# JiQi-da/Mixed-Graph-ADMM

Hardware: AMD Instinct MI355X
Metric: ADMM iters/sec x batch (sample-iterations/s) (higher is better)
Workload: dtype f32; 1 GPU; cfg2: PEMS04-shaped synthetic graph N=307 (path+chords, 340 edges), kNN k=4, T=24, t_in=12; batch_per_gpu=4096, global_batch=4096, ablation=None, graph=kNN-directed, max_cg_iter=100, parallelism=batch-sharded x1, no collective on the convergence path, final RCCL gather, all_finite=True

## Files before the change

mixed-graph-admm_amd/csrc/lds_args.h:

```cpp
#pragma once
#include <hip/hip_runtime.h>

#include "lds_consts.h"
#include "lds_param_table.h"
#include "lds_adapt.h"

struct LdsArgsCore {
    int T, N, TN, TS, t_in, G, B, Bp;
    int nthreads;
    int NR;
    int has_phi, has_zd, first;
    int J;
    int lhsx_kind;
    int band, skip, q1;
    int max_cg;
    int record;
    int stagger_wgs, stagger_ticks;
    int tail_pairs;
    float rho, rho_u, rho_d, mu_u, mu_d1, mu_d2;
    float cx1, cx2;
    double cg_tol2;
    const int* csr;
    int lds_img0, lds_img_ints;
    int off_rp_u, off_rp_d, off_en_u, off_en_d, off_lead_t, off_tail_t;
    int off_diag;
    const float* band_w;
    float *zu, *zd, *phi, *gam, *gu, *gd;
    const float* y;
    const float* mask;
    double* ps;
    int* cg_iters;
    float* alpha_hist;
    float* beta_hist;
    int* nonfinite;
    const int* stop;
};
struct LdsArgs : LdsArgsCore {
    float* xs[LDS_MAXJ + 1];
    int* pstop;
    int* pstop_count;
    float* x_final;
    double admm_tol;
    int it0;
    const LdsSampleParams* sp;
    unsigned long long npos;
    int off_node;
    int img_stride;
    const int* gset;
    int sp_rows{}, sp_row0{}, sp_stride{};
};

struct LdsLaunch {
    int64_t key;
    int block;
    size_t lds_bytes;
    int64_t* instance;
    int* unit;
};

int mg_lds_iteration(const LdsLaunch& L, const LdsArgs& a, int B, hipStream_t st);
int mg_lds_iteration_ps(const LdsLaunch& L, const LdsArgs& a, int B, hipStream_t st);
int mg_lds_iteration_pp(const LdsLaunch& L, const LdsArgs& a, int B, hipStream_t st);
int mg_lds_init(bool masked, int T, int t_in, int N, int TPG, int B, float tm, float den, const float* y, const float* mask, float* x,
                float* zu, float* zd, float* gam, float* gu, float* gd, int* nonfinite, const int* row_of_node, hipStream_t st);
int mg_lds_state_layout(bool to_thread_major, int T, int N, int TPG, int B, const float* src, float* dst, const int* row_of_node, hipStream_t st);
int mg_lds_dxps(int T, int N, int B, const float* x, const float* xo, double* scratch, double* out, const int* stop, hipStream_t st);
int mg_lds_ps_history(const double* ps, const int* pstop, int n_it, int max_it, int B, int Bp, int* n_per_sample, double* metrics,
                      double* out_ps, hipStream_t st);
int mg_lds_stop_test(const double* metrics_row, const int* nonfinite, int has_phi, int has_zd, double tol, int it, int* stop, hipStream_t st);
struct LdsAdaptArgs {
    const double* ps;
    const int* pstop;
    double* w;
    LdsSampleParams* table;
    double* hist;
    int B, Bp, row_first, row_last, ablation, has_phi, has_zd;
    ldsadapt::Params q;
};
int mg_lds_adapt(const LdsAdaptArgs& a, hipStream_t st);
```

mixed-graph-admm_amd/csrc/lds_engine.h:

```cpp
#pragma once
#include <thread>

#include "engine.h"
#include "lds_args.h"
#include "lds_graph_sets.h"
#include "lds_schedule.h"

namespace {

struct LdsEngine final : Engine<float> {
    int dev_cus = 0;
    int* d_lds_csr = nullptr;
    double* d_m2 = nullptr;
    int lds_async = 1;
    int* d_stop = nullptr;
    double* d_ps_ring = nullptr;
    int* d_pstop = nullptr;
    double* d_ps_full = nullptr;
    size_t ps_full_elems = 0;
    LdsSampleParams* d_sp = nullptr;
    LdsSampleParams* d_sch = nullptr;
    size_t sch_elems = 0;
    int sch_up_B = 0;
    LdsSampleParams* d_ad_tab = nullptr;
    double *d_ad_w = nullptr, *d_ad_hist = nullptr;
    size_t ad_tab_elems = 0, ad_w_elems = 0, ad_hist_elems = 0;
    int ad_last_B = 0;
    int* d_sg_img = nullptr;
    int* d_sg_set = nullptr;
    std::vector<int> lds_img_host;
    ldsplan::Switches lds_sw;
    static constexpr int ring_ids[] = {V_XA, V_XB, V_ZUB, V_ZDB, V_PHIB, V_Y, V_MASK, V_R, V_P, V_Q, V_AP, V_RHS, V_TMP, V_IO0, V_IO1};
    static constexpr int NRING = (int)(sizeof(ring_ids) / sizeof(ring_ids[0]));
    std::vector<float*> lds_ring_extra;
    hipStream_t st_side = nullptr;
    hipEvent_t ev_main[LDS_NBOUND] = {nullptr}, ev_side[LDS_NBOUND] = {nullptr};

    using Engine<float>::Engine;
    ~LdsEngine() override {
        (void)hipSetDevice(g->device);
        auto fr = [](void* q) { if (q) (void)hipFree(q); };
        fr(d_lds_csr); fr(d_m2); fr(d_stop); fr(d_ps_ring); fr(d_pstop); fr(d_ps_full);
        fr(d_sp); fr(d_sg_img); fr(d_sg_set); fr(d_sch); fr(d_ad_tab); fr(d_ad_w); fr(d_ad_hist);
        for (float* b : lds_ring_extra) if (b) (void)hipFree(b);
        if (st_side) (void)hipStreamDestroy(st_side);
        for (auto& e : ev_main) if (e) (void)hipEventDestroy(e);
        for (auto& e : ev_side) if (e) (void)hipEventDestroy(e);
    }

    int init() override {
        MG_TRY(init_workspace());
        if (const char* e = getenv("MGADMM_LDS_ASYNC")) lds_async = atoi(e);
        MG_TRY(plan_lds());
        return refused(solvegate::admm_convergence_gate(facts(p), "solver_create"));
    }

    int set_params(const mgadmm_params& np) override {
        const mgadmm_params old = p;
        const int rc = Engine<float>::set_params(np);
        if (p.rho != old.rho || p.rho_u != old.rho_u || p.rho_d != old.rho_d || p.mu_u != old.mu_u || p.mu_d1 != old.mu_d1 ||
            p.mu_d2 != old.mu_d2 || p.ablation != old.ablation)
            sch_up_B = 0;
        MG_TRY(rc);
        return wt.sp_B > 0 ? upload_sample_params(wt.sp_B) : (int)MGADMM_OK;
    }

    int set_sample_params(const mgadmm_sample_params* sp, int B) override {
        MG_TRY(Engine<float>::set_sample_params(sp, B));
        sch_up_B = 0;
        if (wt.sp_B == 0) return MGADMM_OK;
        MG_HIP(hipSetDevice(g->device));
        return upload_sample_params(wt.sp_B);
    }
    int upload_sample_params(int n) {
        std::vector<LdsSampleParams> rec;
        ldsparam::fill_records(wt.source(false, p), p.ablation, n, rec);
        if (!d_sp) MG_HIP(hipMalloc(&d_sp, sizeof(LdsSampleParams) * (size_t)Bmax));
        MG_HIP(hipMemcpy(d_sp, rec.data(), sizeof(LdsSampleParams) * rec.size(), hipMemcpyHostToDevice));
        return MGADMM_OK;
    }

    int set_param_schedule(const mgadmm_param_schedule* sch, int n_rows, int B, int first_row) override {
        MG_HIP(hipSetDevice(g->device));
        if ((sch == nullptr || n_rows == 0) && d_sch) {
            MG_HIP(hipDeviceSynchronize());
            (void)hipFree(d_sch);
            d_sch = nullptr;
            sch_elems = 0;
        }
        MG_TRY(Engine<float>::set_param_schedule(sch, n_rows, B, first_row));
        sch_up_B = 0;
        return MGADMM_OK;
    }
    int upload_param_schedule(int B) {
        if (sch_up_B == B && d_sch) return MGADMM_OK;
        std::vector<LdsSampleParams> rec;
        ldsparam::fill_records(wt.source(true, p), p.ablation, B, rec);
        MG_TRY(grow(d_sch, sch_elems, rec.size()));
        MG_HIP(hipMemcpy(d_sch, rec.data(), sizeof(LdsSampleParams) * rec.size(), hipMemcpyHostToDevice));
        sch_up_B = B;
        return MGADMM_OK;
    }

    int get_adaptive_history(int B, double* rho_hist, int max_periods, int* n_periods) override {
        MG_TRY(Engine<float>::get_adaptive_history(B, rho_hist, max_periods, n_periods));
        if (ad_last_periods == 0 || rho_hist == nullptr || max_periods <= 0) return MGADMM_OK;
        MG_REQUIRE(B == ad_last_B, "get_adaptive_history: the last adaptive_rho solve had B = %d, not %d", ad_last_B, B);
        MG_HIP(hipSetDevice(g->device));
        MG_HIP(hipMemcpy(rho_hist, d_ad_hist, sizeof(double) * 3 * (size_t)B * std::min(max_periods, ad_last_periods), hipMemcpyDeviceToHost));
        return MGADMM_OK;
    }

    int set_sample_graphs(int n_sets, mgadmm_graph* const* graphs, const int32_t* set_of_sample, int B) override {
        MG_HIP(hipSetDevice(g->device));
        if (n_sets == 0 && d_sg_img) {
            MG_HIP(hipDeviceSynchronize());
            (void)hipFree(d_sg_img);
            d_sg_img = nullptr;
        }
        MG_TRY(Engine<float>::set_sample_graphs(n_sets, graphs, set_of_sample, B));
        if (n_sets == 0) return MGADMM_OK;
        std::vector<ldsplan::Input> sets;
        for (int s = 0; s < n_sets; ++s)
            sets.push_back(ldsplan::Input{T, N, false, graphs[s]->transpose_by_gather != 0, graphs[s]->hWu, graphs[s]->hWd, graphs[s]->hWdT});
        std::vector<int> table;
        std::string differs;
        int bad = -1;
        if (!ldssets::build_table(lds, lds_img_host, sets, lds_sw, table, &bad, differs, std::min(8, (int)std::thread::hardware_concurrency()))) {
            mg_set_error("set_sample_graphs: sample_graphs set %d does not share the solver's topology -- %s (a weight that underflowed to 0 and "
                         "was dropped, another k or other neighbour lists?)", bad, differs.c_str());
            return MGADMM_ERR_UNSUPPORTED;
        }
        std::vector<int> set_of((size_t)Bp_max, 0);
        std::copy(set_of_sample, set_of_sample + B, set_of.begin());
        int* fresh = nullptr;
        MG_HIP(hipMalloc(&fresh, sizeof(int) * table.size()));
        if (hipMemcpy(fresh, table.data(), sizeof(int) * table.size(), hipMemcpyHostToDevice) != hipSuccess) {
            (void)hipFree(fresh);
            mg_set_error("set_sample_graphs: upload of the images failed");
            return MGADMM_ERR_HIP;
        }
        if (!d_sg_set) MG_HIP(hipMalloc(&d_sg_set, sizeof(int) * (size_t)Bp_max));
        MG_HIP(hipDeviceSynchronize());
        MG_HIP(hipMemcpy(d_sg_set, set_of.data(), sizeof(int) * set_of.size(), hipMemcpyHostToDevice));
        if (d_sg_img) (void)hipFree(d_sg_img);
        d_sg_img = fresh;
        sg_B = B;
        return MGADMM_OK;
    }

    int plan_lds() {
        if (hipDeviceGetAttribute(&dev_cus, hipDeviceAttributeMultiprocessorCount, g->device) != hipSuccess) { (void)hipGetLastError(); dev_cus = 0; }
        std::vector<int> img;
        const ldsplan::Input in{T, N, g->mode == MGADMM_TEMPORAL_BAND, g->transpose_by_gather != 0, g->hWu, g->hWd, g->hWdT};
        lds_sw = ldsplan::Switches::from_env();
        const ldsplan::Status planned = ldsplan::make(in, lds_sw, lds, img);
        if (planned == ldsplan::ROWS_DO_NOT_FIT) {
            mg_set_error("lds: row plan does not fit its launch word (%d waves)", lds.block / 64);
            return MGADMM_ERR_INVALID;
        }
        if (planned == ldsplan::NO_PLAN) return MGADMM_OK;
        MG_HIP(hipMalloc(&d_lds_csr, sizeof(int) * img.size()));
        MG_HIP(hipMemcpy(d_lds_csr, img.data(), sizeof(int) * img.size(), hipMemcpyHostToDevice));
        lds_img_host = img;
        MG_HIP(hipMalloc(&d_m2, sizeof(double) * T * N * (1 + (size_t)(Bmax + 63) / 64)));
        MG_HIP(hipMalloc(&d_stop, sizeof(int)));
        MG_HIP(hipMemset(d_stop, 0, sizeof(int)));
        MG_HIP(hipMalloc(&d_ps_ring, sizeof(double) * LDS_SETS * LDS_MAXJ * MGADMM_NMETRIC * Bp_max));
        MG_HIP(hipMalloc(&d_pstop, sizeof(int) * (2 * (size_t)Bp_max + 1)));
        {
            int lo = 0, hi = 0;
            MG_HIP(hipDeviceGetStreamPriorityRange(&lo, &hi));
            if (const char* e = getenv("MGADMM_LDS_SIDE_PRIO")) lo = atoi(e) > 0 ? hi : lo;
            MG_HIP(hipStreamCreateWithPriority(&st_side, hipStreamNonBlocking, lo));
            for (auto& e : ev_main) MG_HIP(hipEventCreateWithFlags(&e, hipEventDisableTiming));
            for (auto& e : ev_side) MG_HIP(hipEventCreateWithFlags(&e, hipEventDisableTiming));
        }
        return MGADMM_OK;
    }

    const int* lds_row_of_node() const { return lds.row_order ? d_lds_csr + lds.off_rown : nullptr; }

    int launch_lds(const LdsArgs& a, int B) {
        const bool timed = prof_open(0, 0.0);
        LdsLaunch L{lds.instance, lds.block, lds.lds_bytes, &lds_instance, &lds_unit};
        const int rc = mg_lds_iteration(L, a, B, st);
        if (timed) prof_close();
        return rc;
    }

    struct LdsRun {
        ldssched::Schedule s;
        LdsArgs a;
        int B, Bp;
        bool has_phi, has_zd, record, cold;
        float* xo;
        mgadmm_history* hist;
        int n_done = 0, rc = MGADMM_OK;
        std::vector<int> ad_bounds;
    };

    int lds_ring_reserve(int slots) {
        while (NRING + (int)lds_ring_extra.size() < slots) {
            float* b = nullptr;
            MG_HIP(hipMalloc(&b, vec_elems * sizeof(float)));
            lds_ring_extra.push_back(b);
            ws_bytes += (int64_t)(vec_elems * sizeof(float));
        }
        return MGADMM_OK;
    }
    float* lds_ring(int slot) const { return slot < NRING ? vec[ring_ids[slot]] : lds_ring_extra[slot - NRING]; }
    float* lds_xbuf(const LdsRun& r, int k) const {
        const int slot = r.s.slot_of_iterate(k);
        return slot == ldssched::X_OUT ? r.xo : lds_ring(slot);
    }

    void lds_fill_args(LdsRun& r, const void* y, const void* mask) const {
        LdsArgs& a = r.a;
        a = LdsArgs{};
        a.T = T; a.N = N; a.TN = T * N; a.TS = lds.TS; a.t_in = p.t_in; a.G = lds.G; a.B = r.B; a.Bp = r.Bp;
        a.nthreads = lds.nthreads; a.NR = lds.NR; a.tail_pairs = lds.tail_pairs;
        a.has_phi = r.has_phi; a.has_zd = r.has_zd;
        const LhsDef dx = lhs_def(MGADMM_LHS_X);
        a.lhsx_kind = dx.kind == 1 ? 1 : 0;
        a.cx1 = (float)dx.c1; a.cx2 = (float)dx.c2;
        a.band = g->mode == MGADMM_TEMPORAL_BAND; a.skip = g->skip;
        a.q1 = a.band ? 0 : g->q1;
        a.max_cg = p.max_cg_iter; a.record = r.record ? 1 : 0;
        a.rho = (float)p.rho; a.rho_u = (float)p.rho_u; a.rho_d = (float)p.rho_d;
        a.mu_u = (float)p.mu_u; a.mu_d1 = (float)p.mu_d1; a.mu_d2 = (float)p.mu_d2;
        a.cg_tol2 = p.cg_tol * p.cg_tol;
        a.csr = d_lds_csr; a.lds_img0 = lds.lds_img0; a.lds_img_ints = lds.lds_img_ints;
        a.off_rp_u = lds.off_rp_u; a.off_rp_d = lds.off_rp_d;
        a.off_en_u = lds.off_en_u; a.off_en_d = lds.off_en_d; a.off_lead_t = lds.off_lead_t; a.off_tail_t = lds.off_tail_t; a.off_diag = lds.off_diag;
        a.npos = lds.npos_word; a.off_node = lds.off_node;
        a.band_w = g->band_w;
        a.zu = vec[V_ZUA]; a.zd = vec[V_ZDA]; a.phi = vec[V_PHIA];
        a.gam = vec[V_GAM]; a.gu = vec[V_GU]; a.gd = vec[V_GD];
        const int ncu = dev_cus > 0 ? dev_cus : 256;
        int us = 48;
        if (const char* e = getenv("MGADMM_LDS_STAGGER_US")) us = atoi(e);
        a.stagger_wgs = ncu;
        a.stagger_ticks = (r.B >= 2 * ncu && us > 0) ? us * 100 : 0;
        a.y = (const float*)y; a.mask = (const float*)mask;
        a.alpha_hist = r.record ? d_alpha_hist : nullptr; a.beta_hist = r.record ? d_beta_hist : nullptr;
        a.nonfinite = d_nonfinite;
    }

    int lds_state_in(const LdsRun& r, const void* x0, const mgadmm_state* si) {
        const LdsArgs& a = r.a;
        float* const x = lds_xbuf(r, 0);
        if (!si) {
            float tm, den;
            time_moments(tm, den);
            return mg_lds_init(a.mask != nullptr, T, p.t_in, N, lds.TPG, r.B, tm, den, a.y, a.mask, x, a.zu, a.zd, a.gam, a.gu, a.gd,
                               d_nonfinite, lds_row_of_node(), st);
        }
        if (x0 != nullptr && x != x0) MG_HIP(hipMemcpyAsync(x, x0, (size_t)r.B * T * N * sizeof(float), hipMemcpyDeviceToDevice, st));
        auto in = [&](float* dst, const void* src) {
            return src == nullptr ? (int)MGADMM_OK : mg_lds_state_layout(true, T, N, lds.TPG, r.B, (const float*)src, dst, lds_row_of_node(), st);
        };
        MG_TRY(in(a.zu, si->zu));
        MG_TRY(in(a.gu, si->gamma_u));
        MG_TRY(in(a.zd, si->zd));
        MG_TRY(in(a.gd, si->gamma_d));
        MG_TRY(in(a.phi, si->phi));
        return in(a.gam, si->gamma);
    }
    int lds_state_out(const LdsRun& r, const mgadmm_state* so) {
        const LdsArgs& a = r.a;
        auto out = [&](void* dst, const float* src) {
            return dst == nullptr ? (int)MGADMM_OK : mg_lds_state_layout(false, T, N, lds.TPG, r.B, src, (float*)dst, lds_row_of_node(), st);
        };
        MG_TRY(out(so->zu, a.zu));
        MG_TRY(out(so->zd, a.zd));
        if (r.has_phi) {
            MG_TRY(out(so->phi, a.phi));
            MG_TRY(out(so->gamma, a.gam));
        }
        MG_TRY(out(so->gamma_u, a.gu));
        return out(so->gamma_d, a.gd);
    }

    int lds_batch_metrics(const LdsRun& r, int it, const double* ps, hipStream_t s) {
        const bool per_sample = r.hist && r.hist->metrics_per_sample;
        MG_TRY(mg_lds_dxps(T, N, r.B, lds_xbuf(r, it + 1), lds_xbuf(r, it), d_m2, d_dxps + (size_t)it * T, r.a.stop, s));
        hipLaunchKernelGGL(k_batch_metrics, dim3(MGADMM_NMETRIC), dim3(256), 0, s, ps, r.Bp, r.B, d_hist + (size_t)it * MGADMM_NMETRIC,
                           per_sample ? d_hist_ps + (size_t)it * MGADMM_NMETRIC * r.B : nullptr);
        MG_HIP(hipGetLastError());
        return MGADMM_OK;
    }

    int lagged_word(int c, const int* d_word, int* word) {
        const ldssched::LagStep l = ldssched::lag_step(c, LAG);
        MG_HIP(hipMemcpyAsync(h_flag + 1 + l.put, d_word, sizeof(int), hipMemcpyDeviceToHost, st));
        MG_HIP(hipEventRecord(ev_ring[l.put], st));
        *word = 0;
        if (l.get >= 0) {
            MG_HIP(hipEventSynchronize(ev_ring[l.get]));
            *word = h_flag[1 + l.get];
        }
        return MGADMM_OK;
    }

    int adapt_begin(LdsRun& r) {
        const int B = r.B, max_it = r.s.max_it;
        const ldsparam::Source src = wt.source(false, p);
        std::vector<LdsSampleParams> row, rec;
        ldsparam::fill_records(src, p.ablation, B, row);
        rec.reserve((size_t)max_it * B);
        for (int k = 0; k < max_it; ++k) rec.insert(rec.end(), row.begin(), row.end());
        std::vector<double> w((size_t)ldsparam::NW * B);
        for (int f = 0; f < ldsparam::NW; ++f)
            for (int b = 0; b < B; ++b) w[(size_t)f * B + b] = ldsparam::weight_of(src, f, 0, b);
        const size_t hist_rows = (size_t)max_it / ad.every + 2;
        MG_TRY(grow(d_ad_tab, ad_tab_elems, rec.size()));
        MG_TRY(grow(d_ad_w, ad_w_elems, w.size()));
        MG_TRY(grow(d_ad_hist, ad_hist_elems, hist_rows * 3 * B));
        MG_HIP(hipMemcpy(d_ad_tab, rec.data(), sizeof(LdsSampleParams) * rec.size(), hipMemcpyHostToDevice));
        MG_HIP(hipMemcpy(d_ad_w, w.data(), sizeof(double) * w.size(), hipMemcpyHostToDevice));
        MG_HIP(hipMemcpy(d_ad_hist, w.data(), sizeof(double) * 3 * B, hipMemcpyHostToDevice));
        MG_HIP(hipMemsetAsync(d_ad_hist + (size_t)3 * B, 0xFF, sizeof(double) * (hist_rows - 1) * 3 * B, st));
        ad_last_B = B;
        return MGADMM_OK;
    }
    int adapt_step(LdsRun& r, int it, const double* ps) {
        if (!ad_on || !ldsadapt::step_after(it, ad_start, ad.every, ad.until)) return MGADMM_OK;
        const ldsadapt::Rows rows = ldsadapt::rows_after(it, ad_start, ad.every, ad.until, r.s.max_it);
        r.ad_bounds.push_back(it + 1);
        LdsAdaptArgs k;
        k.ps = ps; k.pstop = r.a.pstop; k.w = d_ad_w; k.table = d_ad_tab;
        k.hist = d_ad_hist + r.ad_bounds.size() * 3 * (size_t)r.B;
        k.B = r.B; k.Bp = r.Bp; k.row_first = rows.first; k.row_last = rows.last;
        k.ablation = p.ablation; k.has_phi = r.has_phi; k.has_zd = r.has_zd;
        k.q = ad;
        return mg_lds_adapt(k, st);
    }

    int lds_run_chunks(LdsRun& r) {
        LdsArgs& a = r.a;
        const size_t row = (size_t)MGADMM_NMETRIC * r.Bp;
        int c = 0;
        for (; c < r.s.chunks(); ++c) {
            const ldssched::Chunk ch = r.s.chunk(c);
            a.first = ch.it0 == 0 && r.cold;
            a.J = ch.Jc;
            for (int k = 0; k <= ch.Jc; ++k) a.xs[k] = lds_xbuf(r, ch.it0 + k);
            a.cg_iters = d_cg_iters + (size_t)ch.it0 * 3 * r.Bp;
            a.it0 = ch.it0;
            if (r.s.per_sample) {
                a.ps = d_ps_full + (size_t)ch.it0 * row;
                MG_TRY(launch_lds(a, r.B));
                MG_TRY(adapt_step(r, ch.it0 + ch.Jc - 1, a.ps + (size_t)(ch.Jc - 1) * row));
                r.n_done = ch.it0 + ch.Jc;
                int stopped = 0;
                MG_TRY(lagged_word(c, a.pstop_count, &stopped));
                if (stopped == r.B) break;
                continue;
            }
            a.ps = d_ps_ring + (size_t)ch.set * r.s.J * row;
            if (ch.wait >= 0) MG_HIP(hipStreamWaitEvent(st, ev_side[ch.wait], 0));
            MG_TRY(launch_lds(a, r.B));
            MG_HIP(hipEventRecord(ev_main[ch.ev], st));
            MG_HIP(hipStreamWaitEvent(st_side, ev_main[ch.ev], 0));
            MG_TRY(adapt_step(r, ch.it0 + ch.Jc - 1, a.ps + (size_t)(ch.Jc - 1) * row));
            for (int k = 0; k < ch.Jc; ++k) MG_TRY(lds_batch_metrics(r, ch.it0 + k, a.ps + (size_t)k * row, st_side));
            MG_HIP(hipEventRecord(ev_side[ch.ev], st_side));
            r.n_done = ch.it0 + ch.Jc;
        }
        if (!r.s.per_sample && r.s.join(c) >= 0) MG_HIP(hipStreamWaitEvent(st, ev_side[r.s.join(c)], 0));
        return MGADMM_OK;
    }

    int lds_run_steps(LdsRun& r) {
        LdsArgs& a = r.a;
        const size_t K = p.max_cg_iter;
        for (int it = 0; it < r.s.max_it; ++it) {
            a.first = it == 0 && r.cold;
            a.J = 1;
            a.xs[0] = lds_xbuf(r, it); a.xs[1] = lds_xbuf(r, it + 1);
            a.cg_iters = d_cg_iters + (size_t)it * 3 * r.Bp;
            a.ps = d_ps;
            a.it0 = it;
            if (r.s.per_sample) a.ps = d_ps_full + (size_t)it * MGADMM_NMETRIC * r.Bp;
            if (r.record) {
                MG_TRY(fill(d_alpha_hist, 3 * K * r.Bp, (float)NAN));
                MG_TRY(fill(d_beta_hist, 3 * K * r.Bp, (float)NAN));
            }
            MG_TRY(launch_lds(a, r.B));
            MG_TRY(adapt_step(r, it, a.ps));
            if (!r.s.per_sample) MG_TRY(lds_batch_metrics(r, it, a.ps, st));
            if (r.record) {
                for (int w = 0; w < 3; ++w)
                    if (w < 2 || r.has_zd) MG_TRY(save_coeffs(r.Bp, r.hist, it, w, r.B, w));
            }
            r.n_done = it + 1;
            if (r.s.per_sample) {
                MG_HIP(hipMemcpyAsync(h_flag + 1, a.pstop_count, sizeof(int), hipMemcpyDeviceToHost, st));
                MG_HIP(hipStreamSynchronize(st));
                if (h_flag[1] == r.B) break;
            } else if (r.s.kind == ldssched::DEVSTOP) {
                int sw = 0;
                MG_TRY(mg_lds_stop_test(d_hist + (size_t)it * MGADMM_NMETRIC, d_nonfinite, r.has_phi, r.has_zd, p.admm_tol, it, d_stop, st));
                MG_TRY(lagged_word(it, d_stop, &sw));
                if (sw != 0) break;
            } else if (p.check_stop) {
                bool stop = false;
                MG_TRY(host_stop_test(it, r.has_phi, r.has_zd, &stop, &r.rc));
                if (stop) break;
            }
        }
        if (r.s.kind == ldssched::DEVSTOP) {
            MG_HIP(hipMemcpyAsync(h_flag + 1, d_stop, sizeof(int), hipMemcpyDeviceToHost, st));
            MG_HIP(hipStreamSynchronize(st));
            const int sw = h_flag[1];
            if (sw > 0) r.n_done = sw;
            else if (sw < 0) { r.n_done = -sw; r.rc = MGADMM_ERR_NONFINITE; }
        }
        return MGADMM_OK;
    }

    int lds_finish_per_sample(LdsRun& r, std::vector<int>& nps) {
        int* const d_nps = d_pstop + Bp_max + 1;
        MG_TRY(mg_lds_ps_history(d_ps_full, d_pstop, r.n_done, r.s.max_it, r.B, r.Bp, d_nps, d_hist,
                                 (r.hist && r.hist->metrics_per_sample) ? d_hist_ps : nullptr, st));
        nps.resize(r.B);
        MG_HIP(hipMemcpyAsync(nps.data(), d_nps, sizeof(int) * r.B, hipMemcpyDeviceToHost, st));
        MG_HIP(hipStreamSynchronize(st));
        r.n_done = *std::max_element(nps.begin(), nps.end());
        return MGADMM_OK;
    }

    int solve_lds(const void* y, const void* mask, int B, const void* x0, const mgadmm_state* state_in, void* x_out,
                  const mgadmm_state* state_out, mgadmm_history* hist) override {
        LdsRun r;
        r.B = B; r.Bp = (B + 63) / 64 * 64;
        r.has_phi = has_phi(); r.has_zd = has_zd();
        r.record = p.record_cg_coeffs && hist && hist->cg_alpha && hist->cg_beta;
        r.cold = !state_in;
        r.hist = hist;
        r.xo = static_cast<float*>(x_out);
        r.s = ldssched::Schedule::pick(lds_async != 0, r.record, p.check_stop != 0, p.admm_convergence == MGADMM_ADMM_PER_SAMPLE,
                                       ad_on ? ldsadapt::adapt_J(ad.every, std::max(1, std::min(lds_chunk, LDS_MAXJ))) : lds_chunk,
                                       p.max_admm_iter);
        const ldssched::Schedule& s = r.s;
        const bool chunked = s.kind == ldssched::CHUNKS;
        MG_TRY(ensure_hist_ps(hist, B));
        MG_HIP(hipMemsetAsync(d_nonfinite, 0, sizeof(int), st));
        MG_HIP(hipMemsetAsync(d_ps, 0, sizeof(double) * MGADMM_NMETRIC * r.Bp, st));
        MG_HIP(hipMemsetAsync(d_cg_iters, 0, sizeof(int) * (size_t)s.max_it * 3 * r.Bp, st));
        if (s.per_sample) {
            MG_TRY(grow(d_ps_full, ps_full_elems, (size_t)s.max_it * MGADMM_NMETRIC * r.Bp));
            MG_HIP(hipMemsetAsync(d_pstop, 0, sizeof(int) * ((size_t)Bp_max + 1), st));
        }
        MG_TRY(lds_ring_reserve(s.slots()));
        lds_fill_args(r, y, mask);
        MG_TRY(lds_state_in(r, x0, state_in));
        if (s.kind == ldssched::DEVSTOP) {
            r.a.stop = d_stop;
            MG_HIP(hipMemsetAsync(d_stop, 0, sizeof(int), st));
        }
        if (chunked && !s.per_sample) MG_HIP(hipMemsetAsync(d_ps_ring, 0, sizeof(double) * LDS_SETS * s.J * MGADMM_NMETRIC * r.Bp, st));
        if (s.per_sample) {
            r.a.pstop = d_pstop; r.a.pstop_count = d_pstop + Bp_max; r.a.x_final = r.xo; r.a.admm_tol = p.admm_tol;
        }
        if (sg_B > 0) {
            r.a.csr = d_sg_img; r.a.img_stride = ldssets::img_stride(lds); r.a.gset = d_sg_set;
        }
        const solvegate::TableChoice tc = solvegate::table_of(set_state(), wt.sch_row0, s.max_it);
        if (tc.scalar_records) MG_TRY(upload_sample_params(B));
        switch (tc.table) {
            case solvegate::TABLE_NONE: break;
            case solvegate::TABLE_SAMPLE: r.a.sp = d_sp; break;
            case solvegate::TABLE_SCHEDULE: MG_TRY(upload_param_schedule(B)); r.a.sp = d_sch; break;
            case solvegate::TABLE_ADAPTIVE: MG_TRY(adapt_begin(r)); r.a.sp = d_ad_tab; break;
        }
        r.a.sp_rows = tc.sp_rows; r.a.sp_row0 = tc.sp_row0; r.a.sp_stride = tc.stride_B ? B : 0;
        MG_TRY(chunked ? lds_run_chunks(r) : lds_run_steps(r));
        std::vector<int> nps;
        if (s.per_sample) MG_TRY(lds_finish_per_sample(r, nps));
        if (ad_on)
            ad_last_periods = 1 + (int)std::count_if(r.ad_bounds.begin(), r.ad_bounds.end(), [&](int n) { return n <= r.n_done; });
        float* const xc = s.per_sample ? r.xo : lds_xbuf(r, r.n_done);
        if (xc != r.xo)
            MG_HIP(hipMemcpyAsync(x_out, xc, (size_t)B * T * N * sizeof(float), hipMemcpyDeviceToDevice, st));
        if (state_out) MG_TRY(lds_state_out(r, state_out));
        return finish_history(hist, r.n_done, B, r.Bp, r.rc, s.per_sample ? nps.data() : nullptr);
    }
};

}
```

mixed-graph-admm_amd/csrc/lds_launch.hip:

```cpp
#define MG_LDS_UNIT 0
#include "lds_dispatch.h"

int mg_lds_iteration(const LdsLaunch& L, const LdsArgs& a, int B, hipStream_t st) {
    if (a.sp != nullptr) return mg_lds_iteration_pp(L, a, B, st);
    return a.pstop != nullptr ? mg_lds_iteration_ps(L, a, B, st) : lds_dispatch(L, a, B, st);
}

int mg_lds_init(bool masked, int T, int t_in, int N, int TPG, int B, float tm, float den, const float* y, const float* mask, float* x,
                float* zu, float* zd, float* gam, float* gu, float* gd, int* nonfinite, const int* row_of_node, hipStream_t st) {
    dim3 grid((N + 255) / 256, B);
    if (masked) hipLaunchKernelGGL((k_init_lds<true>), grid, dim3(256), 0, st, T, t_in, N, TPG, B, tm, den, y, mask, x, zu, zd, gam, gu, gd, nonfinite, row_of_node);
    else hipLaunchKernelGGL((k_init_lds<false>), grid, dim3(256), 0, st, T, t_in, N, TPG, B, tm, den, y, (const float*)nullptr, x, zu, zd, gam, gu, gd, nonfinite, row_of_node);
    MG_HIP(hipGetLastError());
    return MGADMM_OK;
}

int mg_lds_state_layout(bool to_thread_major, int T, int N, int TPG, int B, const float* src, float* dst, const int* row_of_node, hipStream_t st) {
    dim3 grid((T * N + 255) / 256, B);
    if (to_thread_major) hipLaunchKernelGGL((k_state_layout<true>), grid, dim3(256), 0, st, T, N, TPG, src, dst, row_of_node);
    else hipLaunchKernelGGL((k_state_layout<false>), grid, dim3(256), 0, st, T, N, TPG, src, dst, row_of_node);
    MG_HIP(hipGetLastError());
    return MGADMM_OK;
}

int mg_lds_dxps(int T, int N, int B, const float* x, const float* xo, double* scratch, double* out, const int* stop, hipStream_t st) {
    const int TN = T * N, nsl = (B + 63) / 64;
    if (TN % 4 == 0 && ((uintptr_t)x % 16) == 0 && ((uintptr_t)xo % 16) == 0)
        hipLaunchKernelGGL(k_dxps_sm4, dim3((TN / 4 + 63) / 64, nsl), dim3(64), 0, st, TN, B, x, xo, scratch + TN, stop);
    else
        hipLaunchKernelGGL(k_dxps_sm, dim3((TN + 255) / 256, nsl), dim3(256), 0, st, TN, B, x, xo, scratch + TN, stop);
    hipLaunchKernelGGL(k_dxps_sm_mean, dim3((TN + 255) / 256), dim3(256), 0, st, TN, B, nsl, (const double*)(scratch + TN), scratch, stop);
    hipLaunchKernelGGL(k_dxps_sm_final, dim3(T), dim3(256), 0, st, T, N, (const double*)scratch, out, stop);
    MG_HIP(hipGetLastError());
    return MGADMM_OK;
}

int mg_lds_stop_test(const double* metrics_row, const int* nonfinite, int has_phi, int has_zd, double tol, int it, int* stop, hipStream_t st) {
    hipLaunchKernelGGL(k_lds_stop_test, dim3(1), dim3(64), 0, st, metrics_row, nonfinite, has_phi, has_zd, tol, it, stop);
    MG_HIP(hipGetLastError());
    return MGADMM_OK;
}

int mg_lds_ps_history(const double* ps, const int* pstop, int n_it, int max_it, int B, int Bp, int* n_per_sample, double* metrics,
                      double* out_ps, hipStream_t st) {
    hipLaunchKernelGGL(k_lds_ps_history, dim3(n_it, MGADMM_NMETRIC), dim3(256), 0, st, ps, pstop, max_it, B, Bp, n_per_sample, metrics, out_ps);
    MG_HIP(hipGetLastError());
    return MGADMM_OK;
}

__global__ __launch_bounds__(256) void k_lds_adapt(const LdsAdaptArgs a) {
    const int b = blockIdx.x * 256 + threadIdx.x;
    if (b >= a.B) return;
    if (a.pstop != nullptr && a.pstop[b] != 0) return;
    static_assert(MGADMM_M_DUAL_ZD == MGADMM_M_PRI_ZU + 5, "the six residual sums are consecutive metrics");
    double res[6], w[ldsparam::NW];
    for (int k = 0; k < 6; ++k) res[k] = a.ps[(size_t)(MGADMM_M_PRI_ZU + k) * a.Bp + b];
    for (int f = 0; f < ldsparam::NW; ++f) w[f] = a.w[(size_t)f * a.B + b];
    ldsadapt::step(w, res, a.has_phi, a.has_zd, a.q);
    for (int f = 0; f < 3; ++f) {
        a.w[(size_t)f * a.B + b] = w[f];
        a.hist[(size_t)f * a.B + b] = w[f];
    }
    const LdsSampleParams rec = ldsparam::record_of(a.ablation, w);
    for (int row = a.row_first; row < a.row_last; ++row) a.table[(size_t)row * a.B + b] = rec;
}

int mg_lds_adapt(const LdsAdaptArgs& a, hipStream_t st) {
    hipLaunchKernelGGL(k_lds_adapt, dim3((a.B + 255) / 256), dim3(256), 0, st, a);
    MG_HIP(hipGetLastError());
    return MGADMM_OK;
}
```

Before: 3.101 million ADMM sample-iterations/s.

## Fuse per-iteration metric kernels into a two-launch pass with tunable shape

The dx-per-step reduction (previously four kernels: slice pass, mean, final) and the batch-metric kernel are merged into two launches. One is a grid-stride slice-sum pass with an 8-way unrolled batch loop, the other a combined final kernel that finishes both dx and the scalar metrics in one grid. Its workgroup shape can be chosen per call: small 64-thread, optionally grid-capped launches while the side stream overlaps a busy main-stream chunk, and 256 threads otherwise. The aim is fewer side-stream launches and less contention with the main ADMM kernel, at the cost of fewer parallel blocks for the final reduction and slightly different summation order.

```diff
diff --git a/mixed-graph-admm_amd/csrc/lds_args.h b/mixed-graph-admm_amd/csrc/lds_args.h
--- a/mixed-graph-admm_amd/csrc/lds_args.h
+++ b/mixed-graph-admm_amd/csrc/lds_args.h
@@ -64,7 +64,21 @@
 int mg_lds_init(bool masked, int T, int t_in, int N, int TPG, int B, float tm, float den, const float* y, const float* mask, float* x,
                 float* zu, float* zd, float* gam, float* gu, float* gd, int* nonfinite, const int* row_of_node, hipStream_t st);
 int mg_lds_state_layout(bool to_thread_major, int T, int N, int TPG, int B, const float* src, float* dst, const int* row_of_node, hipStream_t st);
-int mg_lds_dxps(int T, int N, int B, const float* x, const float* xo, double* scratch, double* out, const int* stop, hipStream_t st);
+struct LdsMetricArgs {
+    int T, N, B, Bp;
+    const float *x, *xo;
+    double* scratch;
+    double* dxps;
+    const int* stop;
+    const double* ps;
+    double* out;
+    double* out_ps;
+};
+struct LdsMetricShape {
+    int threads;
+    int wgs;
+};
+int mg_lds_metrics(const LdsMetricArgs& a, const LdsMetricShape& shape, hipStream_t st);
 int mg_lds_ps_history(const double* ps, const int* pstop, int n_it, int max_it, int B, int Bp, int* n_per_sample, double* metrics,
                       double* out_ps, hipStream_t st);
 int mg_lds_stop_test(const double* metrics_row, const int* nonfinite, int has_phi, int has_zd, double tol, int it, int* stop, hipStream_t st);
diff --git a/mixed-graph-admm_amd/csrc/lds_engine.h b/mixed-graph-admm_amd/csrc/lds_engine.h
--- a/mixed-graph-admm_amd/csrc/lds_engine.h
+++ b/mixed-graph-admm_amd/csrc/lds_engine.h
@@ -1,4 +1,6 @@
 #pragma once
+#include <stdio.h>
+
 #include <thread>
 
 #include "engine.h"
@@ -11,7 +13,8 @@
 struct LdsEngine final : Engine<float> {
     int dev_cus = 0;
     int* d_lds_csr = nullptr;
-    double* d_m2 = nullptr;
+    double* d_slice_sums = nullptr;
+    LdsMetricShape metric_busy{64, 0}, metric_idle{256, 0};
     int lds_async = 1;
     int* d_stop = nullptr;
     double* d_ps_ring = nullptr;
@@ -40,7 +43,7 @@
     ~LdsEngine() override {
         (void)hipSetDevice(g->device);
         auto fr = [](void* q) { if (q) (void)hipFree(q); };
-        fr(d_lds_csr); fr(d_m2); fr(d_stop); fr(d_ps_ring); fr(d_pstop); fr(d_ps_full);
+        fr(d_lds_csr); fr(d_slice_sums); fr(d_stop); fr(d_ps_ring); fr(d_pstop); fr(d_ps_full);
         fr(d_sp); fr(d_sg_img); fr(d_sg_set); fr(d_sch); fr(d_ad_tab); fr(d_ad_w); fr(d_ad_hist);
         for (float* b : lds_ring_extra) if (b) (void)hipFree(b);
         if (st_side) (void)hipStreamDestroy(st_side);
@@ -163,7 +166,11 @@
         MG_HIP(hipMalloc(&d_lds_csr, sizeof(int) * img.size()));
         MG_HIP(hipMemcpy(d_lds_csr, img.data(), sizeof(int) * img.size(), hipMemcpyHostToDevice));
         lds_img_host = img;
-        MG_HIP(hipMalloc(&d_m2, sizeof(double) * T * N * (1 + (size_t)(Bmax + 63) / 64)));
+        MG_HIP(hipMalloc(&d_slice_sums, sizeof(double) * T * N * ((size_t)(Bmax + 63) / 64)));
+        if (const char* e = getenv("MGADMM_LDS_METRIC_SHAPE")) {
+            int nt = 0, wgs = 0;
+            if (sscanf(e, "%dx%d", &nt, &wgs) == 2 && (nt == 64 || nt == 256 || nt == 512) && wgs >= 0) metric_busy = LdsMetricShape{nt, wgs};
+        }
         MG_HIP(hipMalloc(&d_stop, sizeof(int)));
         MG_HIP(hipMemset(d_stop, 0, sizeof(int)));
         MG_HIP(hipMalloc(&d_ps_ring, sizeof(double) * LDS_SETS * LDS_MAXJ * MGADMM_NMETRIC * Bp_max));
@@ -282,13 +289,15 @@
         return out(so->gamma_d, a.gd);
     }
 
-    int lds_batch_metrics(const LdsRun& r, int it, const double* ps, hipStream_t s) {
+    int lds_batch_metrics(const LdsRun& r, int it, const double* ps, hipStream_t s, bool busy) {
         const bool per_sample = r.hist && r.hist->metrics_per_sample;
-        MG_TRY(mg_lds_dxps(T, N, r.B, lds_xbuf(r, it + 1), lds_xbuf(r, it), d_m2, d_dxps + (size_t)it * T, r.a.stop, s));
-        hipLaunchKernelGGL(k_batch_metrics, dim3(MGADMM_NMETRIC), dim3(256), 0, s, ps, r.Bp, r.B, d_hist + (size_t)it * MGADMM_NMETRIC,
-                           per_sample ? d_hist_ps + (size_t)it * MGADMM_NMETRIC * r.B : nullptr);
-        MG_HIP(hipGetLastError());
-        return MGADMM_OK;
+        LdsMetricArgs m;
+        m.T = T; m.N = N; m.B = r.B; m.Bp = r.Bp;
+        m.x = lds_xbuf(r, it + 1); m.xo = lds_xbuf(r, it);
+        m.scratch = d_slice_sums; m.dxps = d_dxps + (size_t)it * T; m.stop = r.a.stop;
+        m.ps = ps; m.out = d_hist + (size_t)it * MGADMM_NMETRIC;
+        m.out_ps = per_sample ? d_hist_ps + (size_t)it * MGADMM_NMETRIC * r.B : nullptr;
+        return mg_lds_metrics(m, busy ? metric_busy : metric_idle, s);
     }
 
     int lagged_word(int c, const int* d_word, int* word) {
@@ -364,7 +373,8 @@
             MG_HIP(hipEventRecord(ev_main[ch.ev], st));
             MG_HIP(hipStreamWaitEvent(st_side, ev_main[ch.ev], 0));
             MG_TRY(adapt_step(r, ch.it0 + ch.Jc - 1, a.ps + (size_t)(ch.Jc - 1) * row));
-            for (int k = 0; k < ch.Jc; ++k) MG_TRY(lds_batch_metrics(r, ch.it0 + k, a.ps + (size_t)k * row, st_side));
+            const bool busy = c + 1 < r.s.chunks();
+            for (int k = 0; k < ch.Jc; ++k) MG_TRY(lds_batch_metrics(r, ch.it0 + k, a.ps + (size_t)k * row, st_side, busy));
             MG_HIP(hipEventRecord(ev_side[ch.ev], st_side));
             r.n_done = ch.it0 + ch.Jc;
         }
@@ -389,7 +399,7 @@
             }
             MG_TRY(launch_lds(a, r.B));
             MG_TRY(adapt_step(r, it, a.ps));
-            if (!r.s.per_sample) MG_TRY(lds_batch_metrics(r, it, a.ps, st));
+            if (!r.s.per_sample) MG_TRY(lds_batch_metrics(r, it, a.ps, st, false));
             if (r.record) {
                 for (int w = 0; w < 3; ++w)
                     if (w < 2 || r.has_zd) MG_TRY(save_coeffs(r.Bp, r.hist, it, w, r.B, w));
diff --git a/mixed-graph-admm_amd/csrc/lds_launch.hip b/mixed-graph-admm_amd/csrc/lds_launch.hip
--- a/mixed-graph-admm_amd/csrc/lds_launch.hip
+++ b/mixed-graph-admm_amd/csrc/lds_launch.hip
@@ -1,5 +1,6 @@
 #define MG_LDS_UNIT 0
 #include "lds_dispatch.h"
+#include "lds_metric_kernels.h"
 
 int mg_lds_iteration(const LdsLaunch& L, const LdsArgs& a, int B, hipStream_t st) {
     if (a.sp != nullptr) return mg_lds_iteration_pp(L, a, B, st);
@@ -23,14 +24,27 @@
     return MGADMM_OK;
 }
 
-int mg_lds_dxps(int T, int N, int B, const float* x, const float* xo, double* scratch, double* out, const int* stop, hipStream_t st) {
-    const int TN = T * N, nsl = (B + 63) / 64;
-    if (TN % 4 == 0 && ((uintptr_t)x % 16) == 0 && ((uintptr_t)xo % 16) == 0)
-        hipLaunchKernelGGL(k_dxps_sm4, dim3((TN / 4 + 63) / 64, nsl), dim3(64), 0, st, TN, B, x, xo, scratch + TN, stop);
-    else
-        hipLaunchKernelGGL(k_dxps_sm, dim3((TN + 255) / 256, nsl), dim3(256), 0, st, TN, B, x, xo, scratch + TN, stop);
-    hipLaunchKernelGGL(k_dxps_sm_mean, dim3((TN + 255) / 256), dim3(256), 0, st, TN, B, nsl, (const double*)(scratch + TN), scratch, stop);
-    hipLaunchKernelGGL(k_dxps_sm_final, dim3(T), dim3(256), 0, st, T, N, (const double*)scratch, out, stop);
+template <int NT>
+static void lds_metrics_launch(const LdsMetricArgs& a, int wgs, hipStream_t st) {
+    const int TN = a.T * a.N, nsl = (a.B + 63) / 64;
+    const bool vec4 = TN % 4 == 0 && ((uintptr_t)a.x % 16) == 0 && ((uintptr_t)a.xo % 16) == 0;
+    const long long tasks = (long long)(vec4 ? TN / 4 : TN) * nsl;
+    const long long full = (tasks + NT - 1) / NT;
+    const int grid = (int)(wgs > 0 && wgs < full ? wgs : full);
+    if (vec4) hipLaunchKernelGGL((k_lds_metric_pass<4, NT>), dim3(grid), dim3(NT), 0, st, TN, a.B, a.x, a.xo, a.scratch, a.stop);
+    else hipLaunchKernelGGL((k_lds_metric_pass<1, NT>), dim3(grid), dim3(NT), 0, st, TN, a.B, a.x, a.xo, a.scratch, a.stop);
+    constexpr int NF = NT < 256 ? NT : 256;
+    hipLaunchKernelGGL((k_lds_metric_final<NF>), dim3(a.T + MGADMM_NMETRIC), dim3(NF), 0, st, a.T, a.N, a.B, a.Bp, nsl,
+                       (const double*)a.scratch, a.dxps, a.stop, a.ps, a.out, a.out_ps);
+}
+
+int mg_lds_metrics(const LdsMetricArgs& a, const LdsMetricShape& shape, hipStream_t st) {
+    switch (shape.threads) {
+        case 64: lds_metrics_launch<64>(a, shape.wgs, st); break;
+        case 256: lds_metrics_launch<256>(a, shape.wgs, st); break;
+        case 512: lds_metrics_launch<512>(a, shape.wgs, st); break;
+        default: mg_set_error("lds: metric pass with workgroups of %d threads (64, 256 or 512)", shape.threads); return MGADMM_ERR_INVALID;
+    }
     MG_HIP(hipGetLastError());
     return MGADMM_OK;
 }
diff --git a/mixed-graph-admm_amd/csrc/lds_metric_kernels.h b/mixed-graph-admm_amd/csrc/lds_metric_kernels.h
--- /dev/null
+++ b/mixed-graph-admm_amd/csrc/lds_metric_kernels.h
@@ -0,0 +1,100 @@
+#pragma once
+#include "lds_kernels.h"
+
+template <int V, int NT>
+__global__ __launch_bounds__(NT) void k_lds_metric_pass(int TN, int B, const float* __restrict__ x, const float* __restrict__ xo,
+                                                        double* __restrict__ part, const int* __restrict__ stop) {
+    if (stop != nullptr && *stop != 0) return;
+    const int ncol = TN / V, nsl = (B + 63) / 64;
+    const long long total = (long long)ncol * nsl;
+    for (long long q = (long long)blockIdx.x * NT + threadIdx.x; q < total; q += (long long)gridDim.x * NT) {
+        const int sl = (int)(q / ncol), e = (int)(q - (long long)sl * ncol) * V;
+        const int b0 = sl * 64, b1 = min(B, b0 + 64);
+        double* const dst = part + (size_t)sl * TN + e;
+        if constexpr (V == 4) {
+            double s0 = 0.0, s1 = 0.0, s2 = 0.0, s3 = 0.0;
+            int b = b0;
+            for (; b + 8 <= b1; b += 8) {
+                lds_f4 a[8], o[8];
+#pragma unroll
+                for (int u = 0; u < 8; ++u) {
+                    a[u] = *reinterpret_cast<const lds_f4*>(x + (size_t)(b + u) * TN + e);
+                    o[u] = *reinterpret_cast<const lds_f4*>(xo + (size_t)(b + u) * TN + e);
+                }
+#pragma unroll
+                for (int u = 0; u < 8; ++u) {
+                    s0 += (double)a[u].x - (double)o[u].x;
+                    s1 += (double)a[u].y - (double)o[u].y;
+                    s2 += (double)a[u].z - (double)o[u].z;
+                    s3 += (double)a[u].w - (double)o[u].w;
+                }
+            }
+            for (; b < b1; ++b) {
+                const lds_f4 a = *reinterpret_cast<const lds_f4*>(x + (size_t)b * TN + e);
+                const lds_f4 o = *reinterpret_cast<const lds_f4*>(xo + (size_t)b * TN + e);
+                s0 += (double)a.x - (double)o.x;
+                s1 += (double)a.y - (double)o.y;
+                s2 += (double)a.z - (double)o.z;
+                s3 += (double)a.w - (double)o.w;
+            }
+            dst[0] = s0; dst[1] = s1; dst[2] = s2; dst[3] = s3;
+        } else {
+            double s = 0.0;
+            for (int b = b0; b < b1; ++b) s += (double)x[(size_t)b * TN + e] - (double)xo[(size_t)b * TN + e];
+            dst[0] = s;
+        }
+    }
+}
+
+template <int NT>
+__global__ __launch_bounds__(NT) void k_lds_metric_final(int T, int N, int B, int Bp, int nslices, const double* __restrict__ part,
+                                                         double* __restrict__ dxps, const int* __restrict__ stop,
+                                                         const double* __restrict__ ps, double* __restrict__ out,
+                                                         double* __restrict__ out_ps) {
+#pragma clang fp contract(off)
+    __shared__ double sm[256];
+    const int t = blockIdx.x, TN = T * N;
+    const bool is_dx = t < T;
+    if (is_dx && stop != nullptr && *stop != 0) return;
+    const int m = t - T;
+    for (int j = threadIdx.x; j < 256; j += NT) {
+        double acc = 0.0;
+        if (is_dx) {
+            for (int i = j; i < N; i += 256) {
+                const int e = t * N + i;
+                double s = 0.0;
+                int k = 0;
+                for (; k + 8 <= nslices; k += 8) {
+                    double v[8];
+#pragma unroll
+                    for (int u = 0; u < 8; ++u) v[u] = part[(size_t)(k + u) * TN + e];
+#pragma unroll
+                    for (int u = 0; u < 8; ++u) s += v[u];
+                }
+                for (; k < nslices; ++k) s += part[(size_t)k * TN + e];
+                s /= (double)B;
+                acc += s * s;
+            }
+        } else {
+            for (int c = j; c < B; c += 256) {
+                const double v = ps[(size_t)m * Bp + c];
+                acc += v;
+                if (out_ps) out_ps[(size_t)m * B + c] = v;
+            }
+        }
+        sm[j] = acc;
+    }
+    __syncthreads();
+    for (int w = 128; w > 0; w >>= 1) {
+        for (int j = threadIdx.x; j < w; j += NT) sm[j] += sm[j + w];
+        __syncthreads();
+    }
+    if (threadIdx.x == 0) {
+        if (is_dx) dxps[t] = sqrt(sm[0]);
+        else {
+            const double tot = sm[0];
+            const bool is_mean = (m == MGADMM_M_GLR || m == MGADMM_M_DGTV || m == MGADMM_M_DGLR);
+            out[m] = is_mean ? tot / (double)B : sqrt(tot);
+        }
+    }
+}
```

After: 3.140 million ADMM sample-iterations/s, median of 6. 1.3% higher.
